# Epiphany-f/PSL-SLAM

Measured on AMD Instinct MI355X. Metric: frames/sec ORB+line extract+match, 640x480 RGB-D, 1/2/4/8 MI355X, higher is better.
Workload: dtype u8; 1 GPU; configs[2]: 640x480 synthetic structure scene at the configured line load ('sticks': non-overlapping high-contrast bars), ORB 1000/1.2/8 FAST 20/7 + LSD (LSD_REFINE_ADV) / merge / top-200 / LBD + LIL pairing + RGB-D line glue (isLineGood, crossings, planes) extract, SearchByProjection(cur,last) + LSDmatcher::match, frames resident in HBM; scene=sticks, distinct_frames_per_batch=256, streams=1, launcher=none, multi_gpu=single GPU, lsd_refine=LSD_REFINE_ADV, lbd_sample_bytes_per_frame=2654242

## Files before the change

psl-slam_amd/csrc/pslfe_glue.hip:

```cpp
#include <string.h>

#include <vector>

#include "pslfe_internal.h"

#define PSL_GLUE_MAXPTS 21

struct GlueP3 { double x, y, z; };
__device__ __forceinline__ GlueP3 operator+(const GlueP3& a, const GlueP3& b) { return {a.x + b.x, a.y + b.y, a.z + b.z}; }
__device__ __forceinline__ GlueP3 operator-(const GlueP3& a, const GlueP3& b) { return {a.x - b.x, a.y - b.y, a.z - b.z}; }
__device__ __forceinline__ GlueP3 operator*(const GlueP3& a, double s) { return {a.x * s, a.y * s, a.z * s}; }
__device__ __forceinline__ double gdot(const GlueP3& a, const GlueP3& b) { return a.x * b.x + a.y * b.y + a.z * b.z; }
__device__ __forceinline__ double gnorm(const GlueP3& a) { return __dsqrt_rn(a.x * a.x + a.y * a.y + a.z * a.z); }

template <int M, int N>
__device__ __forceinline__ void psl_jacobi_rows(double (&At)[N][M], double (&W)[N], double (&Vt)[N][N]) {
    const double eps = 2.220446049250313e-16 * 10;
    const int max_iter = M > 30 ? M : 30;
    double Wd[N];
#pragma unroll
    for (int i = 0; i < N; ++i) {
        double sd = 0;
#pragma unroll
        for (int k = 0; k < M; ++k) sd += At[i][k] * At[i][k];
// ... 78 lines not shown
        for (int k = 0; k < M; ++k) At[i][k] *= s;
    }
}

__device__ void psl_comp_du(const GlueP3& pt, double f, double* DU) {
    const double J0[3][3] = {{pt.z / f, 0, pt.x / pt.z}, {0, pt.z / f, pt.y / pt.z}, {0, 0, 1}};
    const double c1 = 0.00273, c2 = 0.00074, c3 = -0.00058;
    const double sd = c1 * pt.z * pt.z + c2 * pt.z + c3;
    const double G[3][3] = {{1, 0, 0}, {0, 1, 0}, {0, 0, sd * sd}};
    double JG[3][3], cov[3][3];
#pragma unroll
    for (int i = 0; i < 3; ++i)
#pragma unroll
        for (int j = 0; j < 3; ++j) JG[i][j] = J0[i][0] * G[0][j] + J0[i][1] * G[1][j] + J0[i][2] * G[2][j];
#pragma unroll
    for (int i = 0; i < 3; ++i)
#pragma unroll
        for (int j = 0; j < 3; ++j) cov[i][j] = JG[i][0] * J0[j][0] + JG[i][1] * J0[j][1] + JG[i][2] * J0[j][2];
    double At[3][3], W[3], Vt[3][3];
#pragma unroll
    for (int i = 0; i < 3; ++i)
#pragma unroll
        for (int j = 0; j < 3; ++j) At[i][j] = cov[j][i];
    psl_jacobi_rows<3, 3>(At, W, Vt);
#pragma unroll
    for (int r = 0; r < 3; ++r) {
        const double d = 1 / __dsqrt_rn(W[r]);
#pragma unroll
        for (int c = 0; c < 3; ++c) DU[3 * r + c] = d * At[r][c];
    }
}

__device__ double psl_mah_dist(const double* DU, const GlueP3& pos, const GlueP3& q1, const GlueP3& q2) {
    const double xa = q1.x, ya = q1.y, za = q1.z, xb = q2.x, yb = q2.y, zb = q2.z;
    const double c1 = DU[0], c2 = DU[1], c3 = DU[2], c4 = DU[3], c5 = DU[4], c6 = DU[5], c7 = DU[6], c8 = DU[7], c9 = DU[8];
    const double x1 = pos.x, x2 = pos.y, x3 = pos.z;
    const double term1 = ((c1 * (x1 - xa) + c2 * (x2 - ya) + c3 * (x3 - za)) * (c4 * (x1 - xb) + c5 * (x2 - yb) + c6 * (x3 - zb)) -
                          (c4 * (x1 - xa) + c5 * (x2 - ya) + c6 * (x3 - za)) * (c1 * (x1 - xb) + c2 * (x2 - yb) + c3 * (x3 - zb))),
                 term2 = ((c1 * (x1 - xa) + c2 * (x2 - ya) + c3 * (x3 - za)) * (c7 * (x1 - xb) + c8 * (x2 - yb) + c9 * (x3 - zb)) -
                          (c7 * (x1 - xa) + c8 * (x2 - ya) + c9 * (x3 - za)) * (c1 * (x1 - xb) + c2 * (x2 - yb) + c3 * (x3 - zb))),
                 term3 = ((c4 * (x1 - xa) + c5 * (x2 - ya) + c6 * (x3 - za)) * (c7 * (x1 - xb) + c8 * (x2 - yb) + c9 * (x3 - zb)) -
                          (c7 * (x1 - xa) + c8 * (x2 - ya) + c9 * (x3 - za)) * (c4 * (x1 - xb) + c5 * (x2 - yb) + c6 * (x3 - zb))),
                 term4 = (c1 * (x1 - xa) - c1 * (x1 - xb) + c2 * (x2 - ya) - c2 * (x2 - yb) + c3 * (x3 - za) - c3 * (x3 - zb)),
                 term5 = (c4 * (x1 - xa) - c4 * (x1 - xb) + c5 * (x2 - ya) - c5 * (x2 - yb) + c6 * (x3 - za) - c6 * (x3 - zb)),
                 term6 = (c7 * (x1 - xa) - c7 * (x1 - xb) + c8 * (x2 - ya) - c8 * (x2 - yb) + c9 * (x3 - za) - c9 * (x3 - zb));
    return __dsqrt_rn((term1 * term1 + term2 * term2 + term3 * term3) / (term4 * term4 + term5 * term5 + term6 * term6));
}

__device__ __forceinline__ GlueP3 psl_proj_pt_ln(const GlueP3& P, const GlueP3& mid, const GlueP3& drct) {
    const GlueP3 A = mid, B = mid + drct, AB = B - A, AP = P - A;
    return A + AB * (gdot(AB, AP) / gdot(AB, AB));
}

__device__ int psl_first_arg(double v, unsigned long long mask, bool want_min) {
    const int lane = threadIdx.x & 63;
    const bool in = (mask >> lane) & 1ull;
    double best = in ? v : (want_min ? 1e300 : -1e300);
    int idx = in ? lane : 64;
#pragma unroll
    for (int o = 32; o > 0; o >>= 1) {
        const double ob = __shfl_xor(best, o);
        const int oi = __shfl_xor(idx, o);
        const bool take = want_min ? (ob < best || (ob == best && oi < idx)) : (ob > best || (ob == best && oi < idx));
        if (take) { best = ob; idx = oi; }
    }
    const bool beats = want_min ? best < 100 : best > -100;
    return beats ? idx : (int)__ffsll((long long)mask) - 1;
}

struct GlueLds {
    double pos[PSL_GLUE_MAXPTS][3];
    double DU[PSL_GLUE_MAXPTS][9];
    uint32_t ring[34];
    int idx[PSL_GLUE_MAXPTS + 3];
    int rank[PSL_GLUE_MAXPTS + 3];
    double term[3][24];
};

__device__ __forceinline__ GlueP3 glue_pos(const GlueLds& S, int i) { return {S.pos[i][0], S.pos[i][1], S.pos[i][2]}; }

__device__ bool psl_verify_line(const GlueLds& S, unsigned long long mask, const GlueP3& A, const GlueP3& B, int np) {
    const int lane = threadIdx.x & 63;
    const GlueP3 me = lane < np ? glue_pos(S, lane) : GlueP3{0, 0, 0};
    const double v = gdot(me - A, B - A);
    const int i1 = psl_first_arg(v, mask, true), i2 = psl_first_arg(v, mask, false);
    const GlueP3 C = psl_proj_pt_ln(glue_pos(S, i1), (A + B) * 0.5, B - A);
    const GlueP3 D = psl_proj_pt_ln(glue_pos(S, i2), (A + B) * 0.5, B - A);
    const double cd = gnorm(D - C);
    if (cd < 0.0000000001) return false;
    uint32_t bit = 0;
    if ((mask >> lane) & 1ull) {
        double lambda = gdot(me - C, D - C) / cd / cd;
        lambda = lambda < 0 ? -lambda : lambda;
        bit = lambda >= 1 ? (1u << 9) : (1u << (unsigned int)floor(lambda * 10));
    }
#pragma unroll
    for (int o = 32; o > 0; o >>= 1) bit |= __shfl_xor(bit, o);
    const double sum = (double)__popc(bit);
    return sum / 10 > 0.7;
}

__device__ __forceinline__ void psl_ordered_sum3(GlueLds& S, double t0, double t1, double t2, int m, double* s0, double* s1, double* s2) {
    const int lane = threadIdx.x & 63;
    if (lane < 24) {
        const bool in = lane < m;
        S.term[0][lane] = in ? t0 : 0.0; S.term[1][lane] = in ? t1 : 0.0; S.term[2][lane] = in ? t2 : 0.0;
    }
    __builtin_amdgcn_wave_barrier();
    const double* my = S.term[lane < 3 ? lane : 0];
    double acc = 0;
    for (int t = 0; t < m; t += 8) {
        double v[8];
#pragma unroll
        for (int k = 0; k < 8; ++k) v[k] = my[t + k];
#pragma unroll
        for (int k = 0; k < 8; ++k) acc += v[k];
    }
    __builtin_amdgcn_wave_barrier();
    const int lo = __double2loint(acc), hi = __double2hiint(acc);
    *s0 = __hiloint2double(__builtin_amdgcn_readlane(hi, 0), __builtin_amdgcn_readlane(lo, 0));
    *s1 = __hiloint2double(__builtin_amdgcn_readlane(hi, 1), __builtin_amdgcn_readlane(lo, 1));
    *s2 = __hiloint2double(__builtin_amdgcn_readlane(hi, 2), __builtin_amdgcn_readlane(lo, 2));
}

__device__ void psl_jacobi_wave(GlueLds& S, double a[3], int m, int n, double W[3], double Vt[9]) {
    const double eps = 2.220446049250313e-16 * 10;
    const int max_iter = m > 30 ? m : 30;
    double Wd[3] = {0, 0, 0};
    auto get = [&](const double* v, int i) { return i == 0 ? v[0] : (i == 1 ? v[1] : v[2]); };
    auto put = [&](double* v, int i, double x) { v[0] = i == 0 ? x : v[0]; v[1] = i == 1 ? x : v[1]; v[2] = i == 2 ? x : v[2]; };
    {
        double s0, s1, s2;
        psl_ordered_sum3(S, a[0] * a[0], a[1] * a[1], a[2] * a[2], m, &s0, &s1, &s2);
        Wd[0] = s0; Wd[1] = n > 1 ? s1 : 0.0; Wd[2] = n > 2 ? s2 : 0.0;
    }
    for (int i = 0; i < n; ++i) {
        for (int k = 0; k < n; ++k) Vt[i * 3 + k] = 0;
        Vt[i * 3 + i] = 1;
    }
    const int npairs = n == 3 ? 3 : (n == 2 ? 1 : 0);
    bool have_p = false;
    double p_next = 0;
    for (int iter = 0; iter < max_iter; ++iter) {
        bool changed = false;
        for (int pr = 0; pr < npairs; ++pr) {
            const int i = pr == 2 ? 1 : 0, j = pr == 0 ? 1 : 2;
            const double ai = get(a, i), aj = get(a, j);
            const double aa = get(Wd, i), bb = get(Wd, j);
            double p;
            if (have_p) p = p_next;
            else { double d1, d2; psl_ordered_sum3(S, ai * aj, 0.0, 0.0, m, &p, &d1, &d2); }
            have_p = false;
            if (fabs(p) <= eps * __dsqrt_rn(aa * bb)) continue;
            p *= 2;
            const double beta = aa - bb, gamma = __dsqrt_rn(p * p + beta * beta);
            double c, sn;
            if (beta < 0) {
                const double delta = (gamma - beta) * 0.5;
                sn = __dsqrt_rn(delta / gamma);
                c = p / (gamma * sn * 2);
            } else {
                c = __dsqrt_rn((gamma + beta) / (gamma * 2));
                sn = p / (gamma * c * 2);
            }
            const double t0 = c * ai + sn * aj;
            const double t1 = -sn * ai + c * aj;
            put(a, i, t0); put(a, j, t1);
            const int npr = pr + 1 < npairs ? pr + 1 : 0;
            const int ni = npr == 2 ? 1 : 0, nj = npr == 0 ? 1 : 2;
            double w0, w1;
            psl_ordered_sum3(S, t0 * t0, t1 * t1, get(a, ni) * get(a, nj), m, &w0, &w1, &p_next);
            put(Wd, i, w0); put(Wd, j, w1);
            have_p = true;
            changed = true;
            for (int k = 0; k < n; ++k) {
                const double v0 = c * Vt[i * 3 + k] + sn * Vt[j * 3 + k];
                const double v1 = -sn * Vt[i * 3 + k] + c * Vt[j * 3 + k];
                Vt[i * 3 + k] = v0; Vt[j * 3 + k] = v1;
            }
        }
        if (!changed) break;
    }
    {
        double s0, s1, s2;
        psl_ordered_sum3(S, a[0] * a[0], a[1] * a[1], a[2] * a[2], m, &s0, &s1, &s2);
        Wd[0] = __dsqrt_rn(s0);
        if (n > 1) Wd[1] = __dsqrt_rn(s1);
        if (n > 2) Wd[2] = __dsqrt_rn(s2);
    }
    for (int i = 0; i < n - 1; ++i) {
        int j = i;
        for (int k = i + 1; k < n; ++k)
            if (Wd[j] < Wd[k]) j = k;
        if (i != j) {
            const double t = Wd[i]; Wd[i] = Wd[j]; Wd[j] = t;
            const double u = a[i]; a[i] = a[j]; a[j] = u;
            for (int k = 0; k < n; ++k) { const double v = Vt[i * 3 + k]; Vt[i * 3 + k] = Vt[j * 3 + k]; Vt[j * 3 + k] = v; }
        }
    }
    for (int i = 0; i < n; ++i) {
        W[i] = Wd[i];
        const double sc = Wd[i] > 2.2250738585072014e-308 ? 1 / Wd[i] : 0.;
        a[i] *= sc;
    }
}

__device__ void psl_line_svd(GlueLds& S, unsigned long long mask, const GlueP3& me, GlueP3* mean_out, GlueP3* drct_out) {
    const int lane = threadIdx.x & 63;
    const int n = __popcll(mask);
    if ((mask >> lane) & 1ull) S.rank[__popcll(mask & ((1ull << lane) - 1ull))] = lane;
    __builtin_amdgcn_wave_barrier();
    GlueP3 mean = {0, 0, 0};
    {
        const GlueP3 q = lane < n ? glue_pos(S, S.rank[lane]) : GlueP3{0, 0, 0};
        psl_ordered_sum3(S, q.x, q.y, q.z, n, &mean.x, &mean.y, &mean.z);
    }
    mean = mean * (1.0 / n);
    double W[3], Vt[9], a[3] = {0, 0, 0};
    GlueP3 drct;
    if (n >= 3) {
        if (lane < n) {
            const GlueP3 p = glue_pos(S, S.rank[lane]);
            a[0] = p.x - mean.x; a[1] = p.y - mean.y; a[2] = p.z - mean.z;
        }
        psl_jacobi_wave(S, a, n, 3, W, Vt);
        drct = {Vt[0], Vt[1], Vt[2]};
    } else {
        if (lane < 3) {
            for (int r = 0; r < n; ++r) {
                const GlueP3 p = glue_pos(S, S.rank[r]);
                a[r] = lane == 0 ? p.x - mean.x : (lane == 1 ? p.y - mean.y : p.z - mean.z);
            }
        }
        psl_jacobi_wave(S, a, 3, n, W, Vt);
        const double r0 = a[0];
        drct.x = __hiloint2double(__builtin_amdgcn_readlane(__double2hiint(r0), 0), __builtin_amdgcn_readlane(__double2loint(r0), 0));
        drct.y = __hiloint2double(__builtin_amdgcn_readlane(__double2hiint(r0), 1), __builtin_amdgcn_readlane(__double2loint(r0), 1));
        drct.z = __hiloint2double(__builtin_amdgcn_readlane(__double2hiint(r0), 2), __builtin_amdgcn_readlane(__double2loint(r0), 2));
    }
    __builtin_amdgcn_wave_barrier();
    (void)me;
    *mean_out = mean;
    *drct_out = drct;
}

__device__ void psl_glibc_srand(GlueLds& S, uint32_t seed, int* k) {
    if ((threadIdx.x & 63) == 0) {
        int32_t s[34];
        s[0] = seed == 0 ? 1 : (int32_t)seed;
        for (int i = 1; i < 31; ++i) {
            const long long hi = s[i - 1] / 127773, lo = s[i - 1] % 127773;
            long long word = 16807 * lo - 2836 * hi;
            if (word < 0) word += 2147483647;
            s[i] = (int32_t)word;
        }
        for (int i = 31; i < 34; ++i) s[i] = s[i - 31];
        for (int i = 0; i < 34; ++i) S.ring[i] = (uint32_t)s[i];
        for (int kk = 34; kk < 34 + 310; ++kk) S.ring[kk % 34] = S.ring[(kk - 31) % 34] + S.ring[(kk - 3) % 34];
    }
    *k = 34 + 310;
    __builtin_amdgcn_wave_barrier();
}
__device__ __forceinline__ int psl_glibc_rand_lane0(GlueLds& S, int k) {
    const uint32_t v = S.ring[(k - 31) % 34] + S.ring[(k - 3) % 34];
    S.ring[k % 34] = v;
    return (int)(v >> 1);
}

#ifndef PSL_GOOD_WAVES
#define PSL_GOOD_WAVES 4
#endif
__global__ __launch_bounds__(64, PSL_GOOD_WAVES) void k_line_good(const PslKeyLine* __restrict__ kls, int kl_stride, const int32_t* __restrict__ nkl,
                                                   int nkl_single, const float* __restrict__ depth, int cols, int rows, int dstride,
                                                   size_t dframe, PslCamera cam, uint32_t seed0, double* __restrict__ lines3d,
                                                   float* __restrict__ lineEq) {
    __shared__ GlueLds S;
    const int frame = blockIdx.x, lane = threadIdx.x;
    const int n = min(nkl ? nkl[frame] : nkl_single, kl_stride);
    const PslKeyLine* K = kls + (size_t)frame * kl_stride;
    const float* D = depth + (size_t)frame * dframe;
    double* L3 = lines3d + (size_t)frame * kl_stride * 6;
    float* LE = lineEq + (size_t)frame * kl_stride * 3;
    const float cx = cam.cx, cy = cam.cy;
    const float invfx = 1.0f / cam.fx, invfy = 1.0f / cam.fy;
    for (int i = lane; i < n * 6; i += 64) L3[i] = 0.0;
    for (int i = lane; i < n * 3; i += 64) LE[i] = -1.0f;
    int rk;
    psl_glibc_srand(S, seed0 + (uint32_t)frame, &rk);
    const unsigned long long lt = (1ull << lane) - 1ull;

    for (int i = 0; i < n; ++i) {
        const float spx = K[i].startPointX, spy = K[i].startPointY, epx = K[i].endPointX, epy = K[i].endPointY;
        const float dxf = spx - epx, dyf = spy - epy;
        const double len = __dsqrt_rn((double)dxf * dxf + (double)dyf * dyf);
        const int ilen = (int)len;
        const double numSmp = (double)(ilen < 20 ? ilen : 20);
        if (numSmp == 0) continue;
        bool valid = false;
        GlueP3 p = {0, 0, 0};
        if (lane <= (int)numSmp) {
            const int j = lane;
            const double w1 = 1 - j / numSmp, w2 = j / numSmp;
            const float ax = (float)(spx * w1), ay = (float)(spy * w1), bx = (float)(epx * w2), by = (float)(epy * w2);
            const double ptx = (double)(ax + bx), pty = (double)(ay + by);
            if (!(ptx < 0 || pty < 0 || ptx >= cols || pty >= rows)) {
                int row, col;
                if ((floor(ptx) == ptx) && (floor(pty) == pty)) {
                    col = max((int)(ptx - 1), 0);
                    row = max((int)(pty - 1), 0);
                } else {
                    col = (int)ptx;
                    row = (int)pty;
                }
                const float dv = D[(size_t)row * dstride + col];
                if (!((double)dv <= 0.01)) {
                    valid = true;
                    p.z = dv;
                    p.x = (col - cx) * p.z * invfx;
                    p.y = (row - cy) * p.z * invfy;
                }
            }
        }
        const unsigned long long vmask = __ballot(valid);
        const int np = __popcll(vmask);
        if (np < 5) continue;
        if (valid) {
            const int r = __popcll(vmask & lt);
            S.pos[r][0] = p.x; S.pos[r][1] = p.y; S.pos[r][2] = p.z;
            double DU[9];
            psl_comp_du(p, (double)cam.fx, DU);
#pragma unroll
            for (int c = 0; c < 9; ++c) S.DU[r][c] = DU[c];
        }
        if (lane < np) S.idx[lane] = lane;
        __builtin_amdgcn_wave_barrier();
        const GlueP3 me = lane < np ? glue_pos(S, lane) : GlueP3{0, 0, 0};
        double myDU[9];
#pragma unroll
        for (int c = 0; c < 9; ++c) myDU[c] = lane < np ? S.DU[lane][c] : 0.0;
        const int maxIterNo = min(10, (int)(np * (np - 1) * 0.5));
        const double distThresh = 3.0;
        unsigned long long maxMask = 0;
        int maxCnt = 0, bestA = 0, bestB = 0;
        for (int iter = 0; iter < maxIterNo; ++iter) {
            if (lane == 0) {
                int left = np, begin = 0;
                for (int num = 0; num < 2; ++num) {
                    const int r = begin + psl_glibc_rand_lane0(S, rk + num) % left;
                    const int t = S.idx[begin]; S.idx[begin] = S.idx[r]; S.idx[r] = t;
                    ++begin; --left;
                }
            }
            rk += 2;
            __builtin_amdgcn_wave_barrier();
            const int ia = S.idx[0], ib = S.idx[1];
            const GlueP3 A = glue_pos(S, ia), B = glue_pos(S, ib);
            if (gnorm(B - A) < 0.0000000001) continue;
            const bool in = lane < np && psl_mah_dist(myDU, me, A, B) < distThresh;
            const unsigned long long inMask = __ballot(in);
            const int cnt = __popcll(inMask);
            if (cnt > maxCnt) {
                if (psl_verify_line(S, inMask, A, B, np)) { maxMask = inMask; maxCnt = cnt; bestA = ia; bestB = ib; }
            }
            if (maxCnt > np * 0.6) break;
        }
        GlueP3 outA = {0, 0, 0}, outB = {0, 0, 0};
        if (maxCnt >= 2) {
            GlueP3 m = (glue_pos(S, bestA) + glue_pos(S, bestB)) * 0.5, d = glue_pos(S, bestB) - glue_pos(S, bestA);
            while (true) {
                GlueP3 tm, td;
                psl_line_svd(S, maxMask, me, &tm, &td);
                const bool in = lane < np && psl_mah_dist(myDU, me, tm, tm + td) < distThresh;
                const unsigned long long tmask = __ballot(in);
                if (__popcll(tmask) > maxCnt) { maxMask = tmask; maxCnt = __popcll(tmask); m = tm; d = td; }
                else break;
            }
            const double dp = gdot(me - m, d);
            const int e1 = psl_first_arg(dp, maxMask, true), e2 = psl_first_arg(dp, maxMask, false);
            outA = glue_pos(S, e1);
            outB = glue_pos(S, e2);
        }
        if (gnorm(outA - outB) > 0.02 && lane == 0) {
            const float e0 = (float)(outB.x - outA.x), e1f = (float)(outB.y - outA.y), e2f = (float)(outB.z - outA.z);
            const float magn = sqrtf(e0 * e0 + e1f * e1f + e2f * e2f);
            L3[6 * i] = outA.x; L3[6 * i + 1] = outA.y; L3[6 * i + 2] = outA.z;
            L3[6 * i + 3] = outB.x; L3[6 * i + 4] = outB.y; L3[6 * i + 5] = outB.z;
            LE[3 * i] = e0 / magn; LE[3 * i + 1] = e1f / magn; LE[3 * i + 2] = e2f / magn;
        }
        __builtin_amdgcn_wave_barrier();
    }
}

__global__ __launch_bounds__(64) void k_fans_planes(const PslKeyLine* __restrict__ kls, int kl_stride, const float* __restrict__ fans,
                                                     int fan_stride, const int32_t* __restrict__ nfans_arr, int nfans_single,
                                                     const double* __restrict__ lines3d, const float* __restrict__ lineEq,
                                                     int32_t* __restrict__ pair, float* __restrict__ xy, double* __restrict__ cross,
                                                     int32_t* __restrict__ nint_out, int int_cap, float* __restrict__ planes,
                                                     double* __restrict__ normals, int32_t* __restrict__ lineNo, double* __restrict__ cross3d,
                                                     double* __restrict__ cross2d, double* __restrict__ le_l, int32_t* __restrict__ nplanes_out,
                                                     int plane_cap) {
    const int frame = blockIdx.x, lane = threadIdx.x;
    const int nf = min(nfans_arr ? nfans_arr[frame] : nfans_single, fan_stride);
    const PslKeyLine* K = kls + (size_t)frame * kl_stride;
    const float* F = fans + (size_t)frame * fan_stride * 4;
    const double* L3 = lines3d + (size_t)frame * kl_stride * 6;
    const float* LE = lineEq + (size_t)frame * kl_stride * 3;
    int32_t* PR = pair + (size_t)frame * int_cap * 2;
    float* XY = xy + (size_t)frame * int_cap * 2;
    double* CR = cross + (size_t)frame * int_cap * 3;
    double* LL = le_l + (size_t)frame * int_cap * 6;
    const unsigned long long lt = (1ull << lane) - 1ull;
    int k = 0;
    for (int base = 0; base < nf; base += 64) {
        const int i = base + lane;
        bool ok = false;
        float x = 0, y = 0;
        int i1 = 0, i2 = 0;
        GlueP3 cp = {0, 0, 0};
        if (i < nf) {
            x = F[4 * i]; y = F[4 * i + 1];
            i1 = (int)F[4 * i + 2]; i2 = (int)F[4 * i + 3];
            if (i1 >= 0 && i1 < kl_stride && i2 >= 0 && i2 < kl_stride) {
                const double* A1 = L3 + 6 * i1;
                const double* A2 = L3 + 6 * i2;
                const GlueP3 p1 = {A1[0], A1[1], A1[2]}, p2 = {A2[0], A2[1], A2[2]}, e1 = {A1[3], A1[4], A1[5]}, e2 = {A2[3], A2[4], A2[5]};
                const GlueP3 d1 = e1 - p1, d2 = e2 - p2, p2p1 = p1 - p2;
                const double d11 = gdot(d1, d1), d12 = gdot(d1, d2), d22 = gdot(d2, d2), pd1 = gdot(p2p1, d1), pd2 = gdot(p2p1, d2);
                const double det = d11 * (-d22) - (-d12) * d12;
                if (det != 0) {
                    const double b0 = -pd1, b1 = -pd2;
                    const double x0 = (b0 * (-d22) - (-d12) * b1) / det, x1 = (d11 * b1 - d12 * b0) / det;
                    const GlueP3 root1 = p1 + d1 * x0, root2 = p2 + d2 * x1;
                    cp = (root1 + root2) * 0.5;
                    const GlueP3 mid_x = (p1 + p2) * 0.5, mid_y = (e1 + e2) * 0.5;
                    const double distmid = gnorm(mid_x - mid_y) * 2;
// ... 70 lines not shown
            for (int kk = 0; kk < np && kk < plane_cap; ++kk) {
                const float* pli = PL + 4 * kk;
                const float dd = pl[3] - pli[3];
                const float angle = pl[0] * pli[0] + pl[1] * pli[1] + pl[2] * pli[2];
                if ((double)dd > 0.2 || (double)dd < -0.2) continue;
                if ((double)angle < 0.9397 && (double)angle > -0.9397) continue;
                old = true;
                break;
            }
            if (old) continue;
            if (np < plane_cap) {
                for (int c = 0; c < 4; ++c) PL[4 * np + c] = pl[c];
                for (int c = 0; c < 3; ++c) NN[3 * np + c] = nn[c];
                LN[2 * np] = l1; LN[2 * np + 1] = l2;
                for (int c = 0; c < 3; ++c) C3[3 * np + c] = c3[c];
                C2[2 * np] = XY[2 * i]; C2[2 * np + 1] = XY[2 * i + 1];
            }
            ++np;
        }
        nplanes_out[frame] = np;
    }
}

struct pslfe_glue {
    pslfe_ctx* ctx = nullptr;
    int max_lines = 0, max_fans = 0, max_batch = 0, int_cap = 0, plane_cap = 0;
    int last_nframes = 0;
    double* d_lines3d = nullptr;
    float* d_lineEq = nullptr;
    int32_t* d_pair = nullptr;
    float* d_xy = nullptr;
    double* d_cross = nullptr;
    double* d_le_l = nullptr;
    int32_t* d_nint = nullptr;
    float* d_planes = nullptr;
    double* d_normals = nullptr;
    int32_t* d_lineNo = nullptr;
    double* d_cross3d = nullptr;
    double* d_cross2d = nullptr;
    int32_t* d_nplanes = nullptr;
    PslKeyLine* d_kls = nullptr;
    float* d_fans = nullptr;
    float* d_depth = nullptr;
    size_t depth_cap = 0;
    PslDeviceBuffers mem;
};

static int glue_run(pslfe_glue* g, int nframes, const PslKeyLine* d_kls, int kl_stride, const int32_t* d_nkl, int nkl_single,
                    const float* d_fans, int fan_stride, const int32_t* d_nfans, int nfans_single, const float* d_depth, int w, int h,
                    int dstride, size_t dframe, const PslCamera* cam, uint32_t seed0) {
    hipStream_t st = g->ctx->stream;
    {
        PSL_STAGE_BEGIN(g->ctx, "line.good");
        k_line_good<<<nframes, 64, 0, st>>>(d_kls, kl_stride, d_nkl, nkl_single, d_depth, w, h, dstride, dframe, *cam, seed0, g->d_lines3d,
                                           g->d_lineEq);
        PSL_STAGE_END(g->ctx, "line.good");
    }
    {
        PSL_STAGE_BEGIN(g->ctx, "line.planes");
        k_fans_planes<<<nframes, 64, 0, st>>>(d_kls, kl_stride, d_fans, fan_stride, d_nfans, nfans_single, g->d_lines3d, g->d_lineEq, g->d_pair,
                                             g->d_xy, g->d_cross, g->d_nint, g->int_cap, g->d_planes, g->d_normals, g->d_lineNo, g->d_cross3d,
                                             g->d_cross2d, g->d_le_l, g->d_nplanes, g->plane_cap);
        PSL_STAGE_END(g->ctx, "line.planes");
    }
    PSL_HIP(hipGetLastError());
    g->last_nframes = nframes;
    return PSLFE_OK;
}

extern "C" {

void pslfe_glue_destroy(pslfe_glue* g) {
    if (!g) return;
    (void)hipSetDevice(g->ctx->device);
    (void)hipStreamSynchronize(g->ctx->stream);
    delete g;
}

int pslfe_glue_create(pslfe_ctx* ctx, int max_lines, int max_fans, int max_batch, pslfe_glue** out) {
    PSL_REQUIRE(ctx && out, PSLFE_E_INVALID, "pslfe_glue_create: NULL argument");
    *out = nullptr;
    PSL_REQUIRE(max_lines >= 1 && max_fans >= 1 && max_batch >= 1, PSLFE_E_INVALID, "pslfe_glue_create: max_lines %d max_fans %d max_batch %d",
                max_lines, max_fans, max_batch);
    PSL_HIP(hipSetDevice(ctx->device));
    pslfe_glue* g = new pslfe_glue();
    g->ctx = ctx; g->max_lines = max_lines; g->max_fans = max_fans; g->max_batch = max_batch;
    g->int_cap = max_fans; g->plane_cap = max_fans;
    const size_t F = (size_t)max_batch, L = (size_t)max_lines, I = (size_t)g->int_cap, Pn = (size_t)g->plane_cap;
    PslDeviceBuffers& m = g->mem;
    m.alloc(g->d_lines3d, F * L * 6, "d_lines3d");
    m.alloc(g->d_lineEq, F * L * 3, "d_lineEq");
    m.alloc(g->d_pair, F * I * 2, "d_pair");
    m.alloc(g->d_xy, F * I * 2, "d_xy");
    m.alloc(g->d_cross, F * I * 3, "d_cross");
    m.alloc(g->d_le_l, F * I * 6, "d_le_l");
    m.alloc(g->d_nint, F, "d_nint");
    m.alloc(g->d_planes, F * Pn * 4, "d_planes");
    m.alloc(g->d_normals, F * Pn * 3, "d_normals");
    m.alloc(g->d_lineNo, F * Pn * 2, "d_lineNo");
    m.alloc(g->d_cross3d, F * Pn * 3, "d_cross3d");
    m.alloc(g->d_cross2d, F * Pn * 2, "d_cross2d");
    m.alloc(g->d_nplanes, F, "d_nplanes");
    m.alloc(g->d_kls, L, "d_kls");
    m.alloc(g->d_fans, (size_t)max_fans * 4, "d_fans");
    if (int rc = m.check("pslfe_glue_create")) {
        pslfe_glue_destroy(g);
        return rc;
    }
// ... 107 lines not shown
```

Measured before the change: 32090 frames/s.

## Pack three frames per wavefront in line-good RANSAC kernel via lane groups

The line-good kernel used one 64-lane wave per frame while only about 21 lanes held depth samples. It now splits each wave into three 21-lane groups, each handling its own frame, with group-local shuffles, ballots and broadcasts. Control flow becomes predicated and wave-uniform (glue_any) so that groups can diverge in RANSAC and SVD iterations. This cuts the block count to a third but adds emulated shuffles and lockstep iteration until the slowest group finishes. The per-group LDS scratch sharing looks risky.

```diff
diff --git a/psl-slam_amd/csrc/pslfe_glue.hip b/psl-slam_amd/csrc/pslfe_glue.hip
--- a/psl-slam_amd/csrc/pslfe_glue.hip
+++ b/psl-slam_amd/csrc/pslfe_glue.hip
@@ -154,20 +154,85 @@
     return A + AB * (gdot(AB, AP) / gdot(AB, AB));
 }
 
-__device__ int psl_first_arg(double v, unsigned long long mask, bool want_min) {
+#ifndef PSL_GOOD_WAVES
+#define PSL_GOOD_WAVES 4
+#endif
+#ifndef PSL_GOOD_GROUPS
+#define PSL_GOOD_GROUPS 3
+#endif
+#if PSL_GOOD_GROUPS == 1
+#define PSL_GOOD_LW 64
+#define PSL_GOOD_XOR0 32
+typedef unsigned long long glue_mask_t;
+#elif PSL_GOOD_GROUPS == 2
+#define PSL_GOOD_LW 32
+#define PSL_GOOD_XOR0 16
+typedef uint32_t glue_mask_t;
+#elif PSL_GOOD_GROUPS == 3
+#define PSL_GOOD_LW 21
+#define PSL_GOOD_XOR0 16
+typedef uint32_t glue_mask_t;
+#else
+#error "PSL_GOOD_GROUPS must be 1, 2 or 3"
+#endif
+static_assert(PSL_GOOD_LW >= PSL_GLUE_MAXPTS, "a group holds one lane per depth sample");
+
+struct GlueLane { int g, rl, base; };
+__device__ __forceinline__ GlueLane glue_lane() {
     const int lane = threadIdx.x & 63;
-    const bool in = (mask >> lane) & 1ull;
+#if PSL_GOOD_GROUPS == 1
+    return {0, lane, 0};
+#else
+    const int g = min(lane / PSL_GOOD_LW, PSL_GOOD_GROUPS - 1);
+    return {g, lane - g * PSL_GOOD_LW, g * PSL_GOOD_LW};
+#endif
+}
+__device__ __forceinline__ int glue_popc(unsigned long long m) { return __popcll(m); }
+__device__ __forceinline__ int glue_popc(uint32_t m) { return __popc(m); }
+__device__ __forceinline__ int glue_ffs(unsigned long long m) { return (int)__ffsll((long long)m); }
+__device__ __forceinline__ int glue_ffs(uint32_t m) { return (int)__ffs((int)m); }
+__device__ __forceinline__ glue_mask_t glue_ballot(bool p, const GlueLane& ln) {
+    const unsigned long long b = __ballot(p);
+#if PSL_GOOD_GROUPS == 1
+    return b;
+#else
+    return (glue_mask_t)(b >> ln.base) & (glue_mask_t)((1ull << PSL_GOOD_LW) - 1ull);
+#endif
+}
+__device__ __forceinline__ bool glue_any(bool p) { return __ballot(p) != 0ull; }
+template <class T>
+__device__ __forceinline__ T glue_shfl_xor(T v, int o, const GlueLane& ln, bool* ok) {
+#if PSL_GOOD_GROUPS == 3
+    const int prl = ln.rl ^ o;
+    *ok = prl < PSL_GOOD_LW;
+    return __shfl(v, ln.base + (*ok ? prl : ln.rl));
+#else
+    *ok = true;
+    return __shfl_xor(v, o);
+#endif
+}
+__device__ __forceinline__ int glue_from_first(int v, const GlueLane& ln) {
+#if PSL_GOOD_GROUPS == 3
+    return __shfl(v, ln.base);
+#else
+    return v;
+#endif
+}
+
+__device__ __forceinline__ int psl_first_arg(double v, glue_mask_t mask, bool want_min, const GlueLane& ln) {
+    const bool in = (mask >> ln.rl) & 1;
     double best = in ? v : (want_min ? 1e300 : -1e300);
-    int idx = in ? lane : 64;
-#pragma unroll
-    for (int o = 32; o > 0; o >>= 1) {
-        const double ob = __shfl_xor(best, o);
-        const int oi = __shfl_xor(idx, o);
-        const bool take = want_min ? (ob < best || (ob == best && oi < idx)) : (ob > best || (ob == best && oi < idx));
+    int idx = in ? ln.rl : 64;
+#pragma unroll
+    for (int o = PSL_GOOD_XOR0; o > 0; o >>= 1) {
+        bool ok;
+        const double ob = glue_shfl_xor(best, o, ln, &ok);
+        const int oi = glue_shfl_xor(idx, o, ln, &ok);
+        const bool take = ok && (want_min ? (ob < best || (ob == best && oi < idx)) : (ob > best || (ob == best && oi < idx)));
         if (take) { best = ob; idx = oi; }
     }
     const bool beats = want_min ? best < 100 : best > -100;
-    return beats ? idx : (int)__ffsll((long long)mask) - 1;
+    return glue_from_first(beats ? idx : glue_ffs(mask) - 1, ln);
 }
 
 struct GlueLds {
@@ -177,41 +242,62 @@
     int idx[PSL_GLUE_MAXPTS + 3];
     int rank[PSL_GLUE_MAXPTS + 3];
     double term[3][24];
+    double bc[3];
 };
 
 __device__ __forceinline__ GlueP3 glue_pos(const GlueLds& S, int i) { return {S.pos[i][0], S.pos[i][1], S.pos[i][2]}; }
 
-__device__ bool psl_verify_line(const GlueLds& S, unsigned long long mask, const GlueP3& A, const GlueP3& B, int np) {
-    const int lane = threadIdx.x & 63;
-    const GlueP3 me = lane < np ? glue_pos(S, lane) : GlueP3{0, 0, 0};
+__device__ __forceinline__ void glue_bcast3(GlueLds& S, double x, const GlueLane& ln, double* s0, double* s1, double* s2) {
+#if PSL_GOOD_GROUPS == 1
+    const int lo = __double2loint(x), hi = __double2hiint(x);
+    *s0 = __hiloint2double(__builtin_amdgcn_readlane(hi, 0), __builtin_amdgcn_readlane(lo, 0));
+    *s1 = __hiloint2double(__builtin_amdgcn_readlane(hi, 1), __builtin_amdgcn_readlane(lo, 1));
+    *s2 = __hiloint2double(__builtin_amdgcn_readlane(hi, 2), __builtin_amdgcn_readlane(lo, 2));
+#else
+    if (ln.rl < 3) S.bc[ln.rl] = x;
+    __builtin_amdgcn_wave_barrier();
+    *s0 = S.bc[0]; *s1 = S.bc[1]; *s2 = S.bc[2];
+    __builtin_amdgcn_wave_barrier();
+#endif
+}
+
+__device__ __forceinline__ bool psl_verify_line(const GlueLds& S, glue_mask_t mask, const GlueP3& A, const GlueP3& B, int np, const GlueLane& ln) {
+    const int rl = ln.rl;
+    const GlueP3 me = rl < np ? glue_pos(S, rl) : GlueP3{0, 0, 0};
     const double v = gdot(me - A, B - A);
-    const int i1 = psl_first_arg(v, mask, true), i2 = psl_first_arg(v, mask, false);
+    const int i1 = max(psl_first_arg(v, mask, true, ln), 0), i2 = max(psl_first_arg(v, mask, false, ln), 0);
     const GlueP3 C = psl_proj_pt_ln(glue_pos(S, i1), (A + B) * 0.5, B - A);
     const GlueP3 D = psl_proj_pt_ln(glue_pos(S, i2), (A + B) * 0.5, B - A);
     const double cd = gnorm(D - C);
-    if (cd < 0.0000000001) return false;
     uint32_t bit = 0;
-    if ((mask >> lane) & 1ull) {
+    if ((mask >> rl) & 1) {
         double lambda = gdot(me - C, D - C) / cd / cd;
         lambda = lambda < 0 ? -lambda : lambda;
         bit = lambda >= 1 ? (1u << 9) : (1u << (unsigned int)floor(lambda * 10));
     }
 #pragma unroll
-    for (int o = 32; o > 0; o >>= 1) bit |= __shfl_xor(bit, o);
+    for (int o = PSL_GOOD_XOR0; o > 0; o >>= 1) {
+        bool ok;
+        const uint32_t ob = (uint32_t)glue_shfl_xor((int)bit, o, ln, &ok);
+        bit |= ok ? ob : 0u;
+    }
+    bit = (uint32_t)glue_from_first((int)bit, ln);
     const double sum = (double)__popc(bit);
-    return sum / 10 > 0.7;
-}
-
-__device__ __forceinline__ void psl_ordered_sum3(GlueLds& S, double t0, double t1, double t2, int m, double* s0, double* s1, double* s2) {
-    const int lane = threadIdx.x & 63;
-    if (lane < 24) {
-        const bool in = lane < m;
-        S.term[0][lane] = in ? t0 : 0.0; S.term[1][lane] = in ? t1 : 0.0; S.term[2][lane] = in ? t2 : 0.0;
+    return !(cd < 0.0000000001) && sum / 10 > 0.7;
+}
+
+__device__ __forceinline__ void psl_ordered_sum3(GlueLds& S, double t0, double t1, double t2, int m, const GlueLane& ln, double* s0, double* s1,
+                                                 double* s2) {
+    const int rl = ln.rl;
+    if (rl < 24) {
+        const bool in = rl < m;
+        S.term[0][rl] = in ? t0 : 0.0; S.term[1][rl] = in ? t1 : 0.0; S.term[2][rl] = in ? t2 : 0.0;
     }
     __builtin_amdgcn_wave_barrier();
-    const double* my = S.term[lane < 3 ? lane : 0];
+    const double* my = S.term[rl < 3 ? rl : 0];
+    const int mm = glue_any(m > 16) ? 24 : (glue_any(m > 8) ? 16 : (glue_any(m > 0) ? 8 : 0));
     double acc = 0;
-    for (int t = 0; t < m; t += 8) {
+    for (int t = 0; t < mm; t += 8) {
         double v[8];
 #pragma unroll
         for (int k = 0; k < 8; ++k) v[k] = my[t + k];
@@ -219,41 +305,49 @@
         for (int k = 0; k < 8; ++k) acc += v[k];
     }
     __builtin_amdgcn_wave_barrier();
-    const int lo = __double2loint(acc), hi = __double2hiint(acc);
-    *s0 = __hiloint2double(__builtin_amdgcn_readlane(hi, 0), __builtin_amdgcn_readlane(lo, 0));
-    *s1 = __hiloint2double(__builtin_amdgcn_readlane(hi, 1), __builtin_amdgcn_readlane(lo, 1));
-    *s2 = __hiloint2double(__builtin_amdgcn_readlane(hi, 2), __builtin_amdgcn_readlane(lo, 2));
-}
-
-__device__ void psl_jacobi_wave(GlueLds& S, double a[3], int m, int n, double W[3], double Vt[9]) {
+    glue_bcast3(S, acc, ln, s0, s1, s2);
+}
+
+__device__ __forceinline__ double glue_get3(const double* v, int i) { return i == 0 ? v[0] : (i == 1 ? v[1] : v[2]); }
+__device__ __forceinline__ void glue_put3(double* v, int i, double x) { v[0] = i == 0 ? x : v[0]; v[1] = i == 1 ? x : v[1]; v[2] = i == 2 ? x : v[2]; }
+
+__device__ __forceinline__ void psl_jacobi_wave(GlueLds& S, double a[3], int m, int n, bool on, const GlueLane& ln, double Vt[9]) {
     const double eps = 2.220446049250313e-16 * 10;
-    const int max_iter = m > 30 ? m : 30;
+    const int max_iter = 30;
     double Wd[3] = {0, 0, 0};
-    auto get = [&](const double* v, int i) { return i == 0 ? v[0] : (i == 1 ? v[1] : v[2]); };
-    auto put = [&](double* v, int i, double x) { v[0] = i == 0 ? x : v[0]; v[1] = i == 1 ? x : v[1]; v[2] = i == 2 ? x : v[2]; };
+    m = on ? m : 0;
+    n = on ? n : 0;
     {
         double s0, s1, s2;
-        psl_ordered_sum3(S, a[0] * a[0], a[1] * a[1], a[2] * a[2], m, &s0, &s1, &s2);
+        psl_ordered_sum3(S, a[0] * a[0], a[1] * a[1], a[2] * a[2], m, ln, &s0, &s1, &s2);
         Wd[0] = s0; Wd[1] = n > 1 ? s1 : 0.0; Wd[2] = n > 2 ? s2 : 0.0;
     }
-    for (int i = 0; i < n; ++i) {
-        for (int k = 0; k < n; ++k) Vt[i * 3 + k] = 0;
-        Vt[i * 3 + i] = 1;
-    }
+#pragma unroll
+    for (int i = 0; i < 3; ++i)
+#pragma unroll
+        for (int k = 0; k < 3; ++k) Vt[i * 3 + k] = i == k ? 1 : 0;
     const int npairs = n == 3 ? 3 : (n == 2 ? 1 : 0);
-    bool have_p = false;
+    bool have_p = false, run = on;
     double p_next = 0;
     for (int iter = 0; iter < max_iter; ++iter) {
+        if (!glue_any(run)) break;
         bool changed = false;
-        for (int pr = 0; pr < npairs; ++pr) {
+#pragma unroll
+        for (int pr = 0; pr < 3; ++pr) {
             const int i = pr == 2 ? 1 : 0, j = pr == 0 ? 1 : 2;
-            const double ai = get(a, i), aj = get(a, j);
-            const double aa = get(Wd, i), bb = get(Wd, j);
-            double p;
-            if (have_p) p = p_next;
-            else { double d1, d2; psl_ordered_sum3(S, ai * aj, 0.0, 0.0, m, &p, &d1, &d2); }
-            have_p = false;
-            if (fabs(p) <= eps * __dsqrt_rn(aa * bb)) continue;
+            const bool pact = run && pr < npairs;
+            const double ai = a[i], aj = a[j];
+            const double aa = Wd[i], bb = Wd[j];
+            double p = p_next;
+            const bool need = pact && !have_p;
+            if (glue_any(need)) {
+                double pc, d1, d2;
+                psl_ordered_sum3(S, ai * aj, 0.0, 0.0, need ? m : 0, ln, &pc, &d1, &d2);
+                p = need ? pc : p;
+            }
+            have_p = pact ? false : have_p;
+            const bool rot = pact && !(fabs(p) <= eps * __dsqrt_rn(aa * bb));
+            if (!glue_any(rot)) continue;
             p *= 2;
             const double beta = aa - bb, gamma = __dsqrt_rn(p * p + beta * beta);
             double c, sn;
@@ -267,87 +361,98 @@
             }
             const double t0 = c * ai + sn * aj;
             const double t1 = -sn * ai + c * aj;
-            put(a, i, t0); put(a, j, t1);
-            const int npr = pr + 1 < npairs ? pr + 1 : 0;
-            const int ni = npr == 2 ? 1 : 0, nj = npr == 0 ? 1 : 2;
-            double w0, w1;
-            psl_ordered_sum3(S, t0 * t0, t1 * t1, get(a, ni) * get(a, nj), m, &w0, &w1, &p_next);
-            put(Wd, i, w0); put(Wd, j, w1);
-            have_p = true;
-            changed = true;
-            for (int k = 0; k < n; ++k) {
-                const double v0 = c * Vt[i * 3 + k] + sn * Vt[j * 3 + k];
-                const double v1 = -sn * Vt[i * 3 + k] + c * Vt[j * 3 + k];
-                Vt[i * 3 + k] = v0; Vt[j * 3 + k] = v1;
-            }
-        }
-        if (!changed) break;
+            if (rot) { a[i] = t0; a[j] = t1; }
+            const int nps = pr == 2 ? 0 : pr + 1, nis = nps == 2 ? 1 : 0, njs = nps == 0 ? 1 : 2;
+            const double nprod = npairs == 3 ? a[nis] * a[njs] : a[0] * a[1];
+            double w0, w1, pn;
+            psl_ordered_sum3(S, t0 * t0, t1 * t1, nprod, rot ? m : 0, ln, &w0, &w1, &pn);
+            if (rot) {
+                Wd[i] = w0; Wd[j] = w1;
+                p_next = pn;
+                have_p = true;
+                changed = true;
+#pragma unroll
+                for (int k = 0; k < 3; ++k) {
+                    const double v0 = c * Vt[i * 3 + k] + sn * Vt[j * 3 + k];
+                    const double v1 = -sn * Vt[i * 3 + k] + c * Vt[j * 3 + k];
+                    Vt[i * 3 + k] = v0; Vt[j * 3 + k] = v1;
+                }
+            }
+        }
+        run = run && changed;
     }
     {
         double s0, s1, s2;
-        psl_ordered_sum3(S, a[0] * a[0], a[1] * a[1], a[2] * a[2], m, &s0, &s1, &s2);
+        psl_ordered_sum3(S, a[0] * a[0], a[1] * a[1], a[2] * a[2], m, ln, &s0, &s1, &s2);
         Wd[0] = __dsqrt_rn(s0);
         if (n > 1) Wd[1] = __dsqrt_rn(s1);
         if (n > 2) Wd[2] = __dsqrt_rn(s2);
     }
-    for (int i = 0; i < n - 1; ++i) {
-        int j = i;
-        for (int k = i + 1; k < n; ++k)
-            if (Wd[j] < Wd[k]) j = k;
-        if (i != j) {
-            const double t = Wd[i]; Wd[i] = Wd[j]; Wd[j] = t;
-            const double u = a[i]; a[i] = a[j]; a[j] = u;
-            for (int k = 0; k < n; ++k) { const double v = Vt[i * 3 + k]; Vt[i * 3 + k] = Vt[j * 3 + k]; Vt[j * 3 + k] = v; }
-        }
-    }
-    for (int i = 0; i < n; ++i) {
-        W[i] = Wd[i];
+#pragma unroll
+    for (int i = 0; i < 2; ++i) {
+        if (i < n - 1) {
+            int j = i;
+#pragma unroll
+            for (int k = i + 1; k < 3; ++k)
+                if (k < n && glue_get3(Wd, j) < Wd[k]) j = k;
+            if (i != j) {
+                const double t = Wd[i]; Wd[i] = glue_get3(Wd, j); glue_put3(Wd, j, t);
+                const double u = a[i]; a[i] = glue_get3(a, j); glue_put3(a, j, u);
+#pragma unroll
+                for (int k = 0; k < 3; ++k) {
+                    const double v = Vt[i * 3 + k];
+                    const double w = j == 1 ? Vt[3 + k] : Vt[6 + k];
+                    Vt[i * 3 + k] = w;
+                    if (j == 1) Vt[3 + k] = v; else Vt[6 + k] = v;
+                }
+            }
+        }
+    }
+#pragma unroll
+    for (int i = 0; i < 3; ++i) {
         const double sc = Wd[i] > 2.2250738585072014e-308 ? 1 / Wd[i] : 0.;
-        a[i] *= sc;
-    }
-}
-
-__device__ void psl_line_svd(GlueLds& S, unsigned long long mask, const GlueP3& me, GlueP3* mean_out, GlueP3* drct_out) {
-    const int lane = threadIdx.x & 63;
-    const int n = __popcll(mask);
-    if ((mask >> lane) & 1ull) S.rank[__popcll(mask & ((1ull << lane) - 1ull))] = lane;
+        if (i < n) a[i] *= sc;
+    }
+}
+
+__device__ __forceinline__ void psl_line_svd(GlueLds& S, glue_mask_t mask, bool on, const GlueLane& ln, GlueP3* mean_out, GlueP3* drct_out) {
+    const int rl = ln.rl;
+    mask = on ? mask : (glue_mask_t)0;
+    const int n = glue_popc(mask);
+    if ((mask >> rl) & 1) S.rank[glue_popc(mask & (((glue_mask_t)1 << rl) - (glue_mask_t)1))] = rl;
     __builtin_amdgcn_wave_barrier();
     GlueP3 mean = {0, 0, 0};
     {
-        const GlueP3 q = lane < n ? glue_pos(S, S.rank[lane]) : GlueP3{0, 0, 0};
-        psl_ordered_sum3(S, q.x, q.y, q.z, n, &mean.x, &mean.y, &mean.z);
+        const GlueP3 q = rl < n ? glue_pos(S, S.rank[rl]) : GlueP3{0, 0, 0};
+        psl_ordered_sum3(S, q.x, q.y, q.z, n, ln, &mean.x, &mean.y, &mean.z);
     }
     mean = mean * (1.0 / n);
-    double W[3], Vt[9], a[3] = {0, 0, 0};
-    GlueP3 drct;
-    if (n >= 3) {
-        if (lane < n) {
-            const GlueP3 p = glue_pos(S, S.rank[lane]);
+    double Vt[9], a[3] = {0, 0, 0};
+    const bool tall = n >= 3;
+    if (tall) {
+        if (rl < n) {
+            const GlueP3 p = glue_pos(S, S.rank[rl]);
             a[0] = p.x - mean.x; a[1] = p.y - mean.y; a[2] = p.z - mean.z;
         }
-        psl_jacobi_wave(S, a, n, 3, W, Vt);
-        drct = {Vt[0], Vt[1], Vt[2]};
-    } else {
-        if (lane < 3) {
-            for (int r = 0; r < n; ++r) {
+    } else if (rl < 3) {
+#pragma unroll
+        for (int r = 0; r < 2; ++r)
+            if (r < n) {
                 const GlueP3 p = glue_pos(S, S.rank[r]);
-                a[r] = lane == 0 ? p.x - mean.x : (lane == 1 ? p.y - mean.y : p.z - mean.z);
-            }
-        }
-        psl_jacobi_wave(S, a, 3, n, W, Vt);
-        const double r0 = a[0];
-        drct.x = __hiloint2double(__builtin_amdgcn_readlane(__double2hiint(r0), 0), __builtin_amdgcn_readlane(__double2loint(r0), 0));
-        drct.y = __hiloint2double(__builtin_amdgcn_readlane(__double2hiint(r0), 1), __builtin_amdgcn_readlane(__double2loint(r0), 1));
-        drct.z = __hiloint2double(__builtin_amdgcn_readlane(__double2hiint(r0), 2), __builtin_amdgcn_readlane(__double2loint(r0), 2));
-    }
+                a[r] = rl == 0 ? p.x - mean.x : (rl == 1 ? p.y - mean.y : p.z - mean.z);
+            }
+    }
+    psl_jacobi_wave(S, a, tall ? n : 3, tall ? 3 : n, on, ln, Vt);
+    GlueP3 wide;
+    glue_bcast3(S, a[0], ln, &wide.x, &wide.y, &wide.z);
+    const GlueP3 drct = tall ? GlueP3{Vt[0], Vt[1], Vt[2]} : wide;
     __builtin_amdgcn_wave_barrier();
-    (void)me;
     *mean_out = mean;
     *drct_out = drct;
 }
 
-__device__ void psl_glibc_srand(GlueLds& S, uint32_t seed, int* k) {
-    if ((threadIdx.x & 63) == 0) {
+__device__ void psl_glibc_srand(GlueLds& S, uint32_t seed, int* k, bool first_lane) {
+    if (first_lane) {
         int32_t s[34];
         s[0] = seed == 0 ? 1 : (int32_t)seed;
         for (int i = 1; i < 31; ++i) {
@@ -363,45 +468,51 @@
     *k = 34 + 310;
     __builtin_amdgcn_wave_barrier();
 }
-__device__ __forceinline__ int psl_glibc_rand_lane0(GlueLds& S, int k) {
+__device__ __forceinline__ int psl_glibc_rand_first(GlueLds& S, int k) {
     const uint32_t v = S.ring[(k - 31) % 34] + S.ring[(k - 3) % 34];
     S.ring[k % 34] = v;
     return (int)(v >> 1);
 }
 
-#ifndef PSL_GOOD_WAVES
-#define PSL_GOOD_WAVES 4
-#endif
 __global__ __launch_bounds__(64, PSL_GOOD_WAVES) void k_line_good(const PslKeyLine* __restrict__ kls, int kl_stride, const int32_t* __restrict__ nkl,
-                                                   int nkl_single, const float* __restrict__ depth, int cols, int rows, int dstride,
+                                                   int nkl_single, int nframes, const float* __restrict__ depth, int cols, int rows, int dstride,
                                                    size_t dframe, PslCamera cam, uint32_t seed0, double* __restrict__ lines3d,
                                                    float* __restrict__ lineEq) {
-    __shared__ GlueLds S;
-    const int frame = blockIdx.x, lane = threadIdx.x;
-    const int n = min(nkl ? nkl[frame] : nkl_single, kl_stride);
+    __shared__ GlueLds SS[PSL_GOOD_GROUPS];
+    const GlueLane ln = glue_lane();
+    const int rl = ln.rl;
+    GlueLds& S = SS[ln.g];
+    const bool live = blockIdx.x * PSL_GOOD_GROUPS + ln.g < nframes;
+    const int frame = live ? blockIdx.x * PSL_GOOD_GROUPS + ln.g : 0;
+    const int n = live ? min(nkl ? nkl[frame] : nkl_single, kl_stride) : 0;
     const PslKeyLine* K = kls + (size_t)frame * kl_stride;
     const float* D = depth + (size_t)frame * dframe;
     double* L3 = lines3d + (size_t)frame * kl_stride * 6;
     float* LE = lineEq + (size_t)frame * kl_stride * 3;
     const float cx = cam.cx, cy = cam.cy;
     const float invfx = 1.0f / cam.fx, invfy = 1.0f / cam.fy;
-    for (int i = lane; i < n * 6; i += 64) L3[i] = 0.0;
-    for (int i = lane; i < n * 3; i += 64) LE[i] = -1.0f;
+    if (rl < PSL_GOOD_LW) {
+        for (int i = rl; i < n * 6; i += PSL_GOOD_LW) L3[i] = 0.0;
+        for (int i = rl; i < n * 3; i += PSL_GOOD_LW) LE[i] = -1.0f;
+        for (int i = rl; i < 3 * 24; i += PSL_GOOD_LW) (&S.term[0][0])[i] = 0.0;
+    }
     int rk;
-    psl_glibc_srand(S, seed0 + (uint32_t)frame, &rk);
-    const unsigned long long lt = (1ull << lane) - 1ull;
-
-    for (int i = 0; i < n; ++i) {
-        const float spx = K[i].startPointX, spy = K[i].startPointY, epx = K[i].endPointX, epy = K[i].endPointY;
+    psl_glibc_srand(S, seed0 + (uint32_t)frame, &rk, rl == 0 && live);
+    const glue_mask_t lt = ((glue_mask_t)1 << rl) - (glue_mask_t)1;
+
+    for (int i = 0; glue_any(i < n); ++i) {
+        bool act = i < n;
+        float spx = 0, spy = 0, epx = 0, epy = 0;
+        if (act) { spx = K[i].startPointX; spy = K[i].startPointY; epx = K[i].endPointX; epy = K[i].endPointY; }
         const float dxf = spx - epx, dyf = spy - epy;
         const double len = __dsqrt_rn((double)dxf * dxf + (double)dyf * dyf);
         const int ilen = (int)len;
         const double numSmp = (double)(ilen < 20 ? ilen : 20);
-        if (numSmp == 0) continue;
+        act = act && !(numSmp == 0);
         bool valid = false;
         GlueP3 p = {0, 0, 0};
-        if (lane <= (int)numSmp) {
-            const int j = lane;
+        if (act && rl <= (int)numSmp) {
+            const int j = rl;
             const double w1 = 1 - j / numSmp, w2 = j / numSmp;
             const float ax = (float)(spx * w1), ay = (float)(spy * w1), bx = (float)(epx * w2), by = (float)(epy * w2);
             const double ptx = (double)(ax + bx), pty = (double)(ay + by);
@@ -423,66 +534,76 @@
                 }
             }
         }
-        const unsigned long long vmask = __ballot(valid);
-        const int np = __popcll(vmask);
-        if (np < 5) continue;
-        if (valid) {
-            const int r = __popcll(vmask & lt);
+        const glue_mask_t vmask = glue_ballot(valid, ln);
+        const int np = glue_popc(vmask);
+        act = act && !(np < 5);
+        if (!glue_any(act)) continue;
+        if (valid && act) {
+            const int r = glue_popc(vmask & lt);
             S.pos[r][0] = p.x; S.pos[r][1] = p.y; S.pos[r][2] = p.z;
             double DU[9];
             psl_comp_du(p, (double)cam.fx, DU);
 #pragma unroll
             for (int c = 0; c < 9; ++c) S.DU[r][c] = DU[c];
         }
-        if (lane < np) S.idx[lane] = lane;
+        if (act && rl < np) S.idx[rl] = rl;
         __builtin_amdgcn_wave_barrier();
-        const GlueP3 me = lane < np ? glue_pos(S, lane) : GlueP3{0, 0, 0};
+        const bool mine = act && rl < np;
+        const GlueP3 me = mine ? glue_pos(S, rl) : GlueP3{0, 0, 0};
         double myDU[9];
 #pragma unroll
-        for (int c = 0; c < 9; ++c) myDU[c] = lane < np ? S.DU[lane][c] : 0.0;
-        const int maxIterNo = min(10, (int)(np * (np - 1) * 0.5));
+        for (int c = 0; c < 9; ++c) myDU[c] = mine ? S.DU[rl][c] : 0.0;
+        const int maxIterNo = act ? min(10, (int)(np * (np - 1) * 0.5)) : 0;
         const double distThresh = 3.0;
-        unsigned long long maxMask = 0;
+        glue_mask_t maxMask = 0;
         int maxCnt = 0, bestA = 0, bestB = 0;
-        for (int iter = 0; iter < maxIterNo; ++iter) {
-            if (lane == 0) {
+        bool run = act;
+        for (int iter = 0;; ++iter) {
+            run = run && iter < maxIterNo;
+            if (!glue_any(run)) break;
+            if (run && rl == 0) {
                 int left = np, begin = 0;
                 for (int num = 0; num < 2; ++num) {
-                    const int r = begin + psl_glibc_rand_lane0(S, rk + num) % left;
+                    const int r = begin + psl_glibc_rand_first(S, rk + num) % left;
                     const int t = S.idx[begin]; S.idx[begin] = S.idx[r]; S.idx[r] = t;
                     ++begin; --left;
                 }
             }
-            rk += 2;
+            rk += run ? 2 : 0;
             __builtin_amdgcn_wave_barrier();
-            const int ia = S.idx[0], ib = S.idx[1];
+            const int ia = run ? S.idx[0] : 0, ib = run ? S.idx[1] : 0;
             const GlueP3 A = glue_pos(S, ia), B = glue_pos(S, ib);
-            if (gnorm(B - A) < 0.0000000001) continue;
-            const bool in = lane < np && psl_mah_dist(myDU, me, A, B) < distThresh;
-            const unsigned long long inMask = __ballot(in);
-            const int cnt = __popcll(inMask);
-            if (cnt > maxCnt) {
-                if (psl_verify_line(S, inMask, A, B, np)) { maxMask = inMask; maxCnt = cnt; bestA = ia; bestB = ib; }
-            }
-            if (maxCnt > np * 0.6) break;
+            const bool go = run && !(gnorm(B - A) < 0.0000000001);
+            const bool in = go && mine && psl_mah_dist(myDU, me, A, B) < distThresh;
+            const glue_mask_t inMask = glue_ballot(in, ln);
+            const int cnt = glue_popc(inMask);
+            const bool ask = go && cnt > maxCnt;
+            if (glue_any(ask)) {
+                const bool okl = psl_verify_line(S, ask ? inMask : (glue_mask_t)0, A, B, ask ? np : 0, ln);
+                if (ask && okl) { maxMask = inMask; maxCnt = cnt; bestA = ia; bestB = ib; }
+            }
+            run = run && !(go && maxCnt > np * 0.6);
         }
         GlueP3 outA = {0, 0, 0}, outB = {0, 0, 0};
-        if (maxCnt >= 2) {
+        const bool fit = act && maxCnt >= 2;
+        if (glue_any(fit)) {
             GlueP3 m = (glue_pos(S, bestA) + glue_pos(S, bestB)) * 0.5, d = glue_pos(S, bestB) - glue_pos(S, bestA);
-            while (true) {
+            bool ref = fit;
+            while (glue_any(ref)) {
                 GlueP3 tm, td;
-                psl_line_svd(S, maxMask, me, &tm, &td);
-                const bool in = lane < np && psl_mah_dist(myDU, me, tm, tm + td) < distThresh;
-                const unsigned long long tmask = __ballot(in);
-                if (__popcll(tmask) > maxCnt) { maxMask = tmask; maxCnt = __popcll(tmask); m = tm; d = td; }
-                else break;
+                psl_line_svd(S, maxMask, ref, ln, &tm, &td);
+                const bool in = ref && mine && psl_mah_dist(myDU, me, tm, tm + td) < distThresh;
+                const glue_mask_t tmask = glue_ballot(in, ln);
+                const bool more = ref && glue_popc(tmask) > maxCnt;
+                if (more) { maxMask = tmask; maxCnt = glue_popc(tmask); m = tm; d = td; }
+                ref = more;
             }
             const double dp = gdot(me - m, d);
-            const int e1 = psl_first_arg(dp, maxMask, true), e2 = psl_first_arg(dp, maxMask, false);
-            outA = glue_pos(S, e1);
-            outB = glue_pos(S, e2);
-        }
-        if (gnorm(outA - outB) > 0.02 && lane == 0) {
+            const glue_mask_t emask = fit ? maxMask : (glue_mask_t)0;
+            const int e1 = max(psl_first_arg(dp, emask, true, ln), 0), e2 = max(psl_first_arg(dp, emask, false, ln), 0);
+            if (fit) { outA = glue_pos(S, e1); outB = glue_pos(S, e2); }
+        }
+        if (fit && gnorm(outA - outB) > 0.02 && rl == 0) {
             const float e0 = (float)(outB.x - outA.x), e1f = (float)(outB.y - outA.y), e2f = (float)(outB.z - outA.z);
             const float magn = sqrtf(e0 * e0 + e1f * e1f + e2f * e2f);
             L3[6 * i] = outA.x; L3[6 * i + 1] = outA.y; L3[6 * i + 2] = outA.z;
@@ -659,8 +780,9 @@
     hipStream_t st = g->ctx->stream;
     {
         PSL_STAGE_BEGIN(g->ctx, "line.good");
-        k_line_good<<<nframes, 64, 0, st>>>(d_kls, kl_stride, d_nkl, nkl_single, d_depth, w, h, dstride, dframe, *cam, seed0, g->d_lines3d,
-                                           g->d_lineEq);
+        const int nblocks = (nframes + PSL_GOOD_GROUPS - 1) / PSL_GOOD_GROUPS;
+        k_line_good<<<nblocks, 64, 0, st>>>(d_kls, kl_stride, d_nkl, nkl_single, nframes, d_depth, w, h, dstride, dframe, *cam, seed0,
+                                           g->d_lines3d, g->d_lineEq);
         PSL_STAGE_END(g->ctx, "line.good");
     }
     {
```

Result: faster. 32790 frames/s, median of 6 (+2.2%).
